# LMP88959/Digital-Subband-Video-1

Measured on AMD Instinct MI355X. Metric: encoded Mpixels/sec, 1080p 4:2:0 GOP=12, bit-exact .dsv, higher is better.
Workload: dtype u8/int16+int32 (bit-exact; packed int16 inside a proven range, int32 escape)

## Files before the change

### digital-subband-video-1_amd/csrc/dsvg_dev.hpp

```cpp
#pragma once
#include <hip/hip_runtime.h>
#include <stdint.h>
#include <stddef.h>

#define DSVG_RSU(x, s) (((x) + (1 << (s)) - 1) >> (s))

#define DSVG_GLOBAL __attribute__((address_space(1)))
template <typename T> static __device__ __forceinline__ DSVG_GLOBAL T *dsvg_global(T *p) { return (DSVG_GLOBAL T *)p; }
template <typename T> static __device__ __forceinline__ T dsvg_at(const DSVG_GLOBAL T *base, unsigned idx)
{
    return *reinterpret_cast<const DSVG_GLOBAL T *>(reinterpret_cast<const DSVG_GLOBAL char *>(base) + idx * (unsigned)sizeof(T));
}
typedef unsigned dsvg_u32x2 __attribute__((ext_vector_type(2)));
typedef unsigned dsvg_u32x4 __attribute__((ext_vector_type(4)));
template <typename P> static __device__ __forceinline__ uint2 dsvg_ld2(P p) { const dsvg_u32x2 v = *reinterpret_cast<const DSVG_GLOBAL dsvg_u32x2 *>(p); return make_uint2(v.x, v.y); }
template <typename P> static __device__ __forceinline__ void dsvg_st2(P p, uint2 v) { *reinterpret_cast<DSVG_GLOBAL dsvg_u32x2 *>(p) = dsvg_u32x2{v.x, v.y}; }
typedef unsigned dsvg_u32x4a4 __attribute__((ext_vector_type(4), aligned(4)));
typedef unsigned dsvg_u32x3a4 __attribute__((ext_vector_type(3), aligned(4)));
template <typename P> static __device__ __forceinline__ uint4 dsvg_ld4(P p) { const dsvg_u32x4 v = *reinterpret_cast<const DSVG_GLOBAL dsvg_u32x4 *>(p); return make_uint4(v.x, v.y, v.z, v.w); }
template <typename P> static __device__ __forceinline__ void dsvg_st4(P p, uint4 v) { *reinterpret_cast<DSVG_GLOBAL dsvg_u32x4 *>(p) = dsvg_u32x4{v.x, v.y, v.z, v.w}; }

struct DMV {
    int16_t x, y;
    uint8_t mode, submask, lo_var, lo_tex, high_detail, pad[3];
// ... 53 lines not shown
    unsigned long long total_bits;
    unsigned nruns;
    int dc;
    int overflow;
    int last_chunk;
    int rc;
};
static_assert(sizeof(HzPlaneSum) == 32, "HzPlaneSum travels to the host as 32-byte records");

struct HzParseChunk {
    unsigned long long m0, m1;
    int cbase;
    int prev_end;
};

struct JobDev {
    const uint8_t *src;
    const uint8_t *srcp[3];
    int srcs[3];
    const uint8_t *ref;
    uint8_t *recon;
    uint8_t *xf;
    uint8_t *pred;
    int32_t *coef;
    int32_t *s3, *s1, *s5;
    const DMV *mvs;
    const uint8_t *stable;
    int32_t *nzpos, *nzval;
    HzChunkSum *chunks;
    HzPlaneSum *psum;
    uint8_t *bits;
    size_t bits_off[3], bits_cap[3];
    size_t nz_off[3];
    size_t hz_coef_off[3];
    int chunk_off[3];
    int dec_cnt[3];
    int dec_runs[3], dec_len[3], dec_dc[3];
    long long dec_bitpos[3];
    uint8_t *nzf;
    HzParseChunk *dec_meta[3];
    long long dec_s0[3];
    int dec_npass[3], dec_ncode[3], dec_first_bad[3];
    int16_t *sym;
    uint8_t *pflag;
    uint8_t *cflag;
    unsigned *stat;
    int dec_sym[3];
    int *dec_flag;
    int dec_lim[16];
    int pf_off[3];
    int fused;
    int32_t *llsym;
    int ll_off[3];
    int llq;
    short ext[8];
    HzPlane hz[3];
    int hqp[16];
    int isP;
    int quant;
// ... 186 lines not shown
```

### digital-subband-video-1_amd/csrc/dsvg_pipe.hip

```cpp
#include <stdlib.h>
#include <algorithm>
#include <cstddef>
#include "dsvg_host.hpp"
#include "dsvg_batch_plan.h"
#include <ctime>
extern "C" void dsv1_par_for(int S, void (*fn)(void *ctx, int s, int tid), void *ctx);
extern "C" void dsv1_par_for_long(int S, void (*fn)(void *ctx, int s, int tid), void *ctx);

#define OPCHK(x) do { int rc_ = (x); if (rc_) return rc_; } while (0)

__global__ void k_spin(long long ticks)
{
    const long long t0 = wall_clock64();
    while (wall_clock64() - t0 < ticks) __builtin_amdgcn_s_sleep(16);
}
static bool streams_concurrent(hipStream_t a, hipStream_t b, hipEvent_t e0, hipEvent_t ea, hipEvent_t eb)
{
    const long long T = 10000;
    if (hipEventRecord(e0, a) != hipSuccess || hipStreamWaitEvent(b, e0, 0) != hipSuccess) return true;
    hipLaunchKernelGGL(k_spin, dim3(1), dim3(64), 0, a, T);
    hipLaunchKernelGGL(k_spin, dim3(1), dim3(64), 0, b, T);
    (void)hipEventRecord(ea, a); (void)hipEventRecord(eb, b);
    (void)hipEventSynchronize(ea); (void)hipEventSynchronize(eb);
    float ta = 0, tb = 0;
// ... 96 lines not shown
    Slab src[6], recon, xf, pred;
    int32_t *coef = nullptr, *s3 = nullptr, *s1 = nullptr, *s5 = nullptr, *nzpos = nullptr, *nzval = nullptr;
    HzChunkSum *chunks = nullptr;
    uint8_t *nzf = nullptr;
    int16_t *sym = nullptr;
    std::vector<hipEvent_t> ev_fetch;
    std::vector<short> slot_ext;
    bool no_lazy_border = false;
    bool no_list_pack = false;
    int32_t *llsym = nullptr;
    int ll_off[3] = {0, 0, 0};
    size_t ll_total = 0;
    bool llq = true;
    int16_t *symP = nullptr;
    uint8_t *pflag = nullptr;
    uint8_t *cflag = nullptr;
    unsigned *stat = nullptr;
    bool stats_on = false;
    bool no_patch_kernel = false;
    bool no_dec_sym_I = false;
    bool no_dec_sym = false;
    bool dec_sym_ok[2] = {false, false};
    HzPlaneSum *psum = nullptr;
    uint8_t *bits = nullptr;
    DMV *mvs = nullptr;
    uint8_t *stable = nullptr;
    JobDev *jobs_d = nullptr, *jobs_h = nullptr;
    std::vector<char> slot_isP;
    struct Quality {
        bool on = false;
// ... 203 lines not shown
    if (c->slot_y_d) (void)hipFree(c->slot_y_d);
    if (c->slot_y_h) (void)hipHostFree(c->slot_y_h);
    if (c->slot_cu_d) (void)hipFree(c->slot_cu_d);
    if (c->slot_cv_d) (void)hipFree(c->slot_cv_d);
    if (c->slot_cs_d) (void)hipFree(c->slot_cs_d);
    if (c->slot_cu_h) (void)hipHostFree(c->slot_cu_h);
    if (c->slot_cv_h) (void)hipHostFree(c->slot_cv_h);
    if (c->slot_cs_h) (void)hipHostFree(c->slot_cs_h);
    if (c->dec_flag_d) (void)hipFree(c->dec_flag_d);
    if (c->dec_flag_h) (void)hipHostFree(c->dec_flag_h);
    for (int i = 0; i < 6; i++) c->src[i].release();
    c->recon.release(); c->xf.release(); c->pred.release();
    xres_geo_free(c->xg);
    scale_geo_free(c->osc);
    void *d[] = {c->coef, c->s3, c->s1, c->s5, c->sym, c->nzpos, c->nzval, c->chunks, c->psum, c->bits, c->mvs, c->stable,
                 c->jobs_d, c->mvf, c->aux_tex, c->aux_var, c->csum, c->slots_d, c->luma_sums, c->yuv_stage, c->gtab_d, c->gath_d, c->ltab_d, c->otab_d, c->ingest[0], c->ingest[1], c->dec_d[0], c->dec_d[1], c->dec_meta, c->ilist_d, c->draw_scratch, c->osc_scratch, c->osc_tab_d, c->nzf, c->symP, c->pflag, c->cflag, c->stat, c->llsym, c->rc_state_d, c->rcj_d, (void *)c->xref_d};
    for (void *p : d) if (p) (void)hipFree(p);
    void *hh[] = {c->jobs_h, c->bits_h, c->psum_h, c->mv_h, c->stable_h, c->slots_h, c->luma_h, c->dec_h[0], c->dec_h[1], c->ilist_h, c->gtab_h, c->gath_h, c->aslots_h, c->amv_h, c->rcj_h, (void *)c->xref_h};
    for (void *p : hh) if (p) (void)hipHostFree(p);
    for (auto &q : c->q) { if (q.dev) (void)hipFree(q.dev); if (q.host) (void)hipHostFree(q.host); }
    if (c->st) (void)hipStreamDestroy(c->st);
    for (int i = 0; i < 2; i++) if (c->ev_mark[i]) (void)hipEventDestroy(c->ev_mark[i]);
    if (c->st_l && c->st_l != c->st_a) (void)hipStreamDestroy(c->st_l);
    if (c->ev_l) (void)hipEventDestroy(c->ev_l);
    if (c->st_a) (void)hipStreamDestroy(c->st_a);
    for (int g = 0; g < DSVG_MAX_CODE_STREAMS; g++) {
        if (c->stx[g]) (void)hipStreamDestroy(c->stx[g]);
        if (c->ev_join[g]) (void)hipEventDestroy(c->ev_join[g]);
    }
    if (c->ev_fork) (void)hipEventDestroy(c->ev_fork);
    for (hipEvent_t e : c->ev_fetch) (void)hipEventDestroy(e);
// ... 244 lines not shown
    if ((rc = c->xf.alloc(c->L[0].pitch * (size_t)max_jobs + 4096))) return fail(rc);
    if ((rc = c->pred.alloc(c->L[0].pitch * (size_t)max_jobs + 4096))) return fail(rc);
    const size_t J = (size_t)max_jobs, O = (size_t)out_slots, S = J * (size_t)c->nwin;
    if ((rc = dmalloc(&c->coef, CL.total * J, true))) return fail(rc);
    if ((rc = dmalloc(&c->s3, CL.s3total * J, true))) return fail(rc);
    if ((rc = dmalloc(&c->s1, CL.s1total * J, true))) return fail(rc);
    if ((rc = dmalloc(&c->s5, CL.s5total * J, true))) return fail(rc);
    if ((rc = dmalloc(&c->nzpos, c->nz_total * J, false))) return fail(rc);
    if ((rc = dmalloc(&c->nzval, c->nz_total * J, false))) return fail(rc);
    if ((rc = dmalloc(&c->chunks, (size_t)c->chunks_per_job * J, true))) return fail(rc);
    if ((rc = dmalloc(&c->sym, c->nz_total * J, true))) return fail(rc);
    const size_t DT = 1;
    if ((rc = dmalloc(&c->nzf, (c->nz_total >> 2) * J * DT, true))) return fail(rc);
    if ((rc = dmalloc(&c->symP, c->nz_total * J * DT, true))) return fail(rc);
    if ((rc = dmalloc(&c->pflag, CL.s3total * J, true))) return fail(rc);
    if ((rc = dmalloc(&c->cflag, (size_t)c->chunks_per_job * J * DT, true))) return fail(rc);
    {
        size_t o = 0;
        for (int p = 0; p < 3; p++) { c->ll_off[p] = (int)o; o += ((size_t)CL.w3[p] * CL.h3[p] + 7) & ~(size_t)7; }
        c->ll_total = o;
        if ((rc = dmalloc(&c->llsym, c->ll_total * J * DT, true))) return fail(rc);
    }
    c->llq = !getenv("DSV1_NO_LLQ");
    if ((rc = dmalloc(&c->stat, 8 * 64, true))) return fail(rc);
    if ((rc = dmalloc(&c->psum, 3 * O, true))) return fail(rc);
    if ((rc = dmalloc(&c->bits, c->bits_per_job * O, true))) return fail(rc);
    if ((rc = dmalloc(&c->mvs, (size_t)c->nblk * O, true))) return fail(rc);
    if ((rc = dmalloc(&c->stable, (size_t)c->nblk * O, true))) return fail(rc);
    if ((rc = dmalloc(&c->jobs_d, O, true))) return fail(rc);
    c->rc_slots = c->bgeo.rc_slots;
// ... 661 lines not shown
            dsvg_ctx *c = B.c;
            const BatchPlan &P = *B.P;
            const int k = idx % P.njobs, d = P.base + idx;
            const dsvg_pic_job &j = B.jobs[idx - k + P.order[(size_t)idx]];
            const int isP = j.ref_recon_slot >= 0;
            JobDev &jb = c->jobs_h[d];
            fill_job(c, jb, k, isP, j.quant, d);
            jb.fused = 1;
            jb.llq = c->llq ? 1 : 0;
            const size_t kk = (size_t)k;
            jb.llsym = c->llsym + kk * c->ll_total;
            for (int p = 0; p < 3; p++) jb.ll_off[p] = c->ll_off[p];
            jb.cflag = c->cflag + kk * c->chunks_per_job;
            jb.nzf = isP ? c->nzf + kk * (c->nz_total >> 2) : nullptr;
            if (isP) jb.sym = c->symP + kk * c->nz_total;
            jb.psum = c->psum + (size_t)j.out_slot * 3;
            jb.bits = c->bits + (size_t)j.out_slot * c->bits_per_job;
            jb.src = c->src[0].p + (size_t)j.src_slot * c->L[0].pitch;
            jb.srcp[0] = jb.src + c->L[0].off[0]; jb.srcs[0] = c->L[0].stride[0];
            if (c->slot_y[(size_t)j.src_slot]) { jb.srcp[0] = c->slot_y[(size_t)j.src_slot]; jb.srcs[0] = c->L[0].w[0]; }
            jb.srcp[1] = c->slot_cu[(size_t)j.src_slot]; jb.srcp[2] = c->slot_cv[(size_t)j.src_slot]; jb.srcs[1] = jb.srcs[2] = c->slot_cs[(size_t)j.src_slot];
            jb.ref = isP ? c->recon.p + (size_t)j.ref_recon_slot * c->L[0].pitch : nullptr;
            jb.recon = j.recon_slot >= 0 ? c->recon.p + (size_t)j.recon_slot * c->L[0].pitch : nullptr;
            if (isP && jb.recon && j.recon_slot != j.ref_recon_slot && !c->no_inplace_pred) jb.pred = jb.recon;
            const size_t um = (size_t)P.base + (size_t)P.mvu[(size_t)idx], us = (size_t)P.base + (size_t)P.stu[(size_t)idx];
            jb.mvs = c->mvs + um * c->nblk;
            jb.stable = c->stable + us * c->nblk;
            if (P.stcp[(size_t)idx]) memcpy(c->stable_h + us * c->nblk, j.stable_blocks, (size_t)c->nblk);
            if (P.mvcp[(size_t)idx]) memcpy(c->mv_h + um * c->nblk, j.mvs, (size_t)c->nblk * sizeof(DMV));
            memcpy(jb.ext, &P.ext[(size_t)idx * 8], sizeof(short) * 8);
// ... 881 lines not shown
```

### digital-subband-video-1_amd/csrc/k_sbt.hip

```cpp
#include <type_traits>
#include "dsvg_dev.hpp"
#include <algorithm>
#include "dsvg_kernels.hpp"
#include "dsvg_host.hpp"

template <int M>
static __device__ __forceinline__ void store_row(int32_t *p, const int (&v)[M], int n)
{
    if (n >= M) {
        if (M == 4 && (((uintptr_t)p) & 15) == 0) {
            *reinterpret_cast<int4 *>(p) = make_int4(v[0], v[1 % M], v[2 % M], v[3 % M]);
            return;
        }
        if (M == 2 && (((uintptr_t)p) & 7) == 0) {
            *reinterpret_cast<int2 *>(p) = make_int2(v[0], v[1 % M]);
            return;
        }
#pragma unroll
        for (int i = 0; i < M; i++) p[i] = v[i];
    } else {
#pragma unroll
        for (int i = 0; i < M; i++)
            if (i < n) p[i] = v[i];
    }
}

struct QCtx {
    const HzPlane *hp;
    const DSVG_GLOBAL uint8_t *stable;
    DSVG_GLOBAL int16_t *sym;
    bool any_ov;
    DSVG_GLOBAL uint8_t *nzf = nullptr, *cfl = nullptr;
    mutable int nz_any = 0;
    __device__ __forceinline__ void put_sparse(int pos, int v) const
    {
        sym[pos] = (int16_t)v;
        nzf[pos >> 2] = 1;
        cfl[pos >> 11] = 1;
    }
};
static_assert(HZ_CHUNK == 2048, "cfl index");
struct QLevel {
    int qp;
    int sh0, sh1;
    int dbx, dby, sw, base0, base1, base2;
};
template <int HZL>
static __device__ __forceinline__ QLevel q_level(const HzPlane &hp)
{
    const HzRegion &r = hp.r[1 + 3 * HZL];
    QLevel L;
    L.qp = r.qp; L.sh0 = r.qp; L.sh1 = r.qp_h;
    L.dbx = r.dbx; L.dby = r.dby; L.sw = r.sw;
    L.base0 = r.base; L.base1 = hp.r[2 + 3 * HZL].base; L.base2 = hp.r[3 + 3 * HZL].base;
    return L;
// ... 230 lines not shown
        }
        if (rowok) {
            const int pr = cy * L.sw + cx0;
            if (q.nzf) {
                int any = 0;
#pragma unroll
                for (int i = 0; i < M; i++) any |= (i < nR ? slh[i] : 0) | ((hasB && i < nC) ? shl[i] : 0) | ((hasB && i < nR) ? shh[i] : 0);
                if (any) {
                    q.nz_any = 1;
#pragma unroll
                    for (int i = 0; i < M; i++) {
                        if (i < nR && slh[i] != 0) q.put_sparse(L.base0 + pr + i, slh[i]);
                        if (hasB && i < nC && shl[i] != 0) q.put_sparse(L.base1 + pr + i, shl[i]);
                        if (hasB && i < nR && shh[i] != 0) q.put_sparse(L.base2 + pr + i, shh[i]);
                    }
                }
            } else {
                store_sym_row<M>(q.sym + L.base0 + pr, slh, nR);
                if (hasB) {
                    store_sym_row<M>(q.sym + L.base1 + pr, shl, nC);
                    store_sym_row<M>(q.sym + L.base2 + pr, shh, nR);
                }
            }
        }
    }
};
template <int N, int HZL>
static __device__ __forceinline__ void haar_fwd_patch_q(const int (&in)[N][N], int (&out)[N / 2][N / 2],
                                                        int cx0, int cy0, int ws, int hs, int W,
                                                        int wo, int ho, int32_t *__restrict__ coef, bool scaled,
// ... 32 lines not shown
            a[r][i + 4] = (int)((v.y >> (8 * i)) & 0xff) - 128;
        }
    }
    const int W = g.W, H = g.H;
    const int wo1 = DSVG_RSU(W, 1), ho1 = DSVG_RSU(H, 1), wo2 = DSVG_RSU(W, 2), ho2 = DSVG_RSU(H, 2);
    int l1[4][4], l2[2][2], l3[1][1];
    QCtx q;
    if (Q) {
        const HzPlane &hp = jb.hz[c];
        q.hp = &hp; q.stable = dsvg_global(jb.stable);
        q.sym = dsvg_global(jb.sym + jb.nz_off[c]);
        q.any_ov = (2 * hp.s_w[0] > hp.s_w[1]) || (2 * hp.s_h[0] > hp.s_h[1]) ||
                   (2 * hp.s_w[1] > hp.s_w[2]) || (2 * hp.s_h[1] > hp.s_h[2]);
        q.nzf = jb.nzf ? dsvg_global(jb.nzf + (jb.nz_off[c] >> 2)) : nullptr;
        q.cfl = jb.nzf ? dsvg_global(jb.cflag + jb.chunk_off[c]) : nullptr;
    }
    if (Q) {
        haar_fwd_patch_q<8, 2>(a, l1, 4 * I, 4 * J, W, H, W, wo1, ho1, coef, false, q);
        haar_fwd_patch_q<4, 1>(l1, l2, 2 * I, 2 * J, wo1, ho1, W, wo2, ho2, coef, true, q);
        haar_fwd_patch_q<2, 0>(l2, l3, I, J, wo2, ho2, W, g.w3, g.h3, coef, true, q);
    } else {
        haar_fwd_patch<8>(a, l1, 4 * I, 4 * J, W, H, W, wo1, ho1, coef, false);
        haar_fwd_patch<4>(l1, l2, 2 * I, 2 * J, wo1, ho1, W, wo2, ho2, coef, true);
        haar_fwd_patch<2>(l2, l3, I, J, wo2, ho2, W, g.w3, g.h3, coef, true);
    }
    jb.s3[g.s3off + (size_t)J * g.w3 + I] = l3[0][0];
    if (Q && jb.nzf) jb.pflag[g.s3off + (size_t)J * g.w3 + I] = (uint8_t)q.nz_any;
}

struct __attribute__((aligned(4))) U4A4 { unsigned x, y, z, w; };

typedef short s16x2 __attribute__((ext_vector_type(2)));
static __device__ __forceinline__ s16x2 pk2(int a, int b) { return s16x2{(short)a, (short)b}; }
static __device__ __forceinline__ s16x2 pk_min(s16x2 a, s16x2 b) { return __builtin_elementwise_min(a, b); }
static __device__ __forceinline__ s16x2 pk_max(s16x2 a, s16x2 b) { return __builtin_elementwise_max(a, b); }
static __device__ __forceinline__ s16x2 pk_rdiv2(s16x2 v) { return (v + (short)1 + (v >> 15)) >> 1; }
static __device__ __forceinline__ s16x2 pk_rdiv4(s16x2 v) { return (v + (short)2 + (v >> 15)) >> 2; }
static __device__ __forceinline__ s16x2 pk_div4(s16x2 v) { return (v + ((v >> 15) & (short)3)) >> 2; }
struct PkRow { s16x2 e0, e1, o0, o1; };
static __device__ __forceinline__ s16x2 pk_u(unsigned v) { return __builtin_bit_cast(s16x2, v); }
static __device__ __forceinline__ unsigned pk_b(s16x2 v) { return __builtin_bit_cast(unsigned, v); }
#define PK_EVEN(hi_, lo_) pk_u((lo_) & 0x00ff00ffu)
// ... 265 lines not shown
    int slh[4], shl[4], shh[4], any = 0;
#pragma unroll
    for (int i = 0; i < 4; i++) {
        const int s0 = r0[2 * i] + r0[2 * i + 1], s1 = r1[2 * i] + r1[2 * i + 1];
        const int d0 = r0[2 * i] - r0[2 * i + 1], d1 = r1[2 * i] - r1[2 * i + 1];
        out[i] = s0 + s1;
        slh[i] = sym_shift(d0 + d1, sh1); shl[i] = sym_shift(s0 - s1, sh1); shh[i] = sym_shift(d0 - d1, sh1);
        any |= slh[i] | shl[i] | shh[i];
    }
    if (any) {
        q.nz_any = 1;
        const int pr = cy1 * L1.sw + cx1;
        put_row4(q, L1.base0 + pr, slh[0], slh[1], slh[2], slh[3]);
        put_row4(q, L1.base1 + pr, shl[0], shl[1], shl[2], shl[3]);
        put_row4(q, L1.base2 + pr, shh[0], shh[1], shh[2], shh[3]);
    }
}
static __device__ __forceinline__ void fwd_fast_rows1_pk(const QCtx &q, const QLevel &L1, int sh1, int cx1, int cy1,
                                                         const PkRow &r0, const PkRow &r1, int (&out)[4])
{
    const s16x2 s0a = r0.e0 + r0.o0, s0b = r0.e1 + r0.o1, d0a = r0.e0 - r0.o0, d0b = r0.e1 - r0.o1;
    const s16x2 s1a = r1.e0 + r1.o0, s1b = r1.e1 + r1.o1, d1a = r1.e0 - r1.o0, d1b = r1.e1 - r1.o1;
    const s16x2 lla = s0a + s1a, llb = s0b + s1b;
    const s16x2 lha = d0a + d1a, lhb = d0b + d1b, hla = s0a - s1a, hlb = s0b - s1b, hha = d0a - d1a, hhb = d0b - d1b;
    out[0] = lla.x; out[1] = lla.y; out[2] = llb.x; out[3] = llb.y;
    const s16x2 mx = pk_max(pk_max(pk_max(lha, lhb), pk_max(hla, hlb)), pk_max(hha, hhb));
    const s16x2 mn = pk_min(pk_min(pk_min(lha, lhb), pk_min(hla, hlb)), pk_min(hha, hhb));
    const s16x2 am = pk_max(mx, s16x2{0, 0} - mn);
    if ((pk_b(am) & ~(((1u << min(sh1, 15)) - 1u) * 0x00010001u)) == 0) return;
    q.nz_any = 1;
    const int pr = cy1 * L1.sw + cx1;
    const short ms = (short)((1 << sh1) - 1), ss = (short)sh1;
    const s16x2 mm = {ms, ms}, sv = {ss, ss}, s15 = {15, 15};
    auto pks = [&](s16x2 v) { return (v + ((v >> s15) & mm)) >> sv; };
    put_row4(q, L1.base0 + pr, pks(lha), pks(lhb));
    put_row4(q, L1.base1 + pr, pks(hla), pks(hlb));
    put_row4(q, L1.base2 + pr, pks(hha), pks(hhb));
}
template <int N, int HZL>
static __device__ __forceinline__ void fwd_fast_level(const QCtx &q, const QLevel &L, const int (&qqv)[N / 2], const float (&rcv)[N / 2], int cx0, int cy0,
                                                      const int (&in)[N][N], int (&out)[N / 2][N / 2])
{
#pragma unroll
    for (int j = 0; j < N / 2; j++)
#pragma unroll
        for (int i = 0; i < N / 2; i++) {
            const int qq = qqv[j];
            const float rc = rcv[j];
            const int a = in[2 * j][2 * i], b = in[2 * j][2 * i + 1], c = in[2 * j + 1][2 * i], d = in[2 * j + 1][2 * i + 1];
            const int s0 = a + b, s1 = c + d, d0 = a - b, d1 = c - d;
            out[j][i] = d_ll_down(s0 + s1);
            const int vlh = d0 + d1, vhl = s0 - s1, vhh = d0 - d1;
#ifndef FWD_FAST_NO_QTEST
            if (max(max(max(vlh, vhl), vhh), -min(min(vlh, vhl), vhh)) < qq) continue;
#endif
            int slh, shl, shh;
            (void)q_coef<HZL>(qq, rc, vlh, slh);
            (void)q_coef<HZL>(qq, rc, vhl, shl);
            (void)q_coef<HZL>(qq, rc, vhh, shh);
            if (slh | shl | shh) {
                q.nz_any = 1;
                const int pr = (cy0 + j) * L.sw + cx0 + i;
                if (slh) q.put_sparse(L.base0 + pr, slh);
                if (shl) q.put_sparse(L.base1 + pr, shl);
                if (shh) q.put_sparse(L.base2 + pr, shh);
            }
        }
}

#ifndef FWD_FAST_INTRA
#define FWD_FAST_INTRA 1
#endif
struct FwdFastSel { bool ok, intra; QLevel L1, L2, L3; int i1[4], i2[2], i3; };
struct FwdFastHp { QLevel L1, L2, L3; int nbh; bool ovx, ovy, sparse; };
static __device__ __forceinline__ FwdFastHp fwd_fast_hp(const JobDev &jb, const HzPlane &hp)
{
    FwdFastHp H;
    const int sw0 = hp.s_w[0], sw1 = hp.s_w[1], sw2 = hp.s_w[2], sh0 = hp.s_h[0], sh1 = hp.s_h[1], sh2 = hp.s_h[2];
    H.L1 = q_level<2>(hp); H.L2 = q_level<1>(hp); H.L3 = q_level<0>(hp);
    H.nbh = hp.nbh;
// ... 55 lines not shown
    FWD_PIN(H.L1.sh0); FWD_PIN(H.L1.sh1); FWD_PIN(H.L1.dbx); FWD_PIN(H.L1.dby); FWD_PIN(H.L2.qp); FWD_PIN(H.L2.dbx); FWD_PIN(H.L2.dby);
    FWD_PIN(H.L3.qp); FWD_PIN(H.L3.dbx); FWD_PIN(H.L3.dby); FWD_PIN(H.nbh); FWD_PIN(mvtab); FWD_PIN(stable_p); FWD_PIN(srcp_p); FWD_PIN(sstride);
#endif
    DMV mv;
    {
        const auto mq = reinterpret_cast<const DSVG_GLOBAL char *>(dsvg_global(mvs0 ? mvs0 + (size_t)job * nblk : mvtab)) + (unsigned)blk * (unsigned)sizeof(DMV);
        const unsigned xy = *reinterpret_cast<const DSVG_GLOBAL unsigned *>(mq);
        mv.x = (int16_t)(xy & 0xffffu); mv.y = (int16_t)(xy >> 16); mv.mode = *reinterpret_cast<const DSVG_GLOBAL uint8_t *>(mq + 4);
    }
    QCtx q;
    q.hp = &hp; q.stable = dsvg_global(stable_p);
    q.sym = dsvg_global(jb.sym + jb.nz_off[c]);
    q.any_ov = H.ovx | H.ovy;
    q.nzf = H.sparse ? dsvg_global(jb.nzf + (jb.nz_off[c] >> 2)) : nullptr;
    q.cfl = H.sparse ? dsvg_global(jb.cflag + jb.chunk_off[c]) : nullptr;
    const FwdFastSel S = fwd_fast_sel(H, mv.mode, I, J, x0, y0, pw, ph);
    if (!S.ok) return;
    const QLevel &L1 = S.L1, &L2 = S.L2, &L3 = S.L3;
    const auto sp = dsvg_global(srcp_p);
    uint2 sw[8];
    if (S.intra) {
        const auto px = dsvg_global(static_cast<const uint8_t *>(jb.xf + g.poff));
#pragma unroll
        for (int r = 0; r < 8; r++) sw[r] = dsvg_ld2(px + (unsigned)((y0 + r) * stride + x0));
    } else {
#pragma unroll
        for (int r = 0; r < 8; r++) sw[r] = dsvg_ld2(sp + (unsigned)((y0 + r) * sstride + x0));
    }
    int f1[4], f2[2];
#pragma unroll
// ... 78 lines not shown
#endif
#pragma unroll
    for (int j = 0; j < 2; j++) {
        fq.q2[j] = max(L2.qp >> ((f2[j] & 2) ? 2 : (f2[j] != 0)), HZ_MINQ);
        fq.rc2[j] = __builtin_amdgcn_rcpf((float)(fq.q2[j] << 1));
    }
    fq.q3 = max(L3.qp >> ((f3 & 2) ? 2 : (f3 != 0)), HZ_MINQ);
    fq.rc3 = __builtin_amdgcn_rcpf((float)(fq.q3 << 1));
    int l2[2][2], l3[1][1];
    fwd_fast_level<4, 1>(q, L2, fq.q2, fq.rc2, 2 * I, 2 * J, l1, l2);
    const int q3v[1] = {fq.q3};
    const float rc3v[1] = {fq.rc3};
    fwd_fast_level<2, 0>(q, L3, q3v, rc3v, I, J, l2, l3);
    dsvg_global(jb.s3 + g.s3off)[(unsigned)(J * g.w3 + I)] = l3[0][0];
    dsvg_global(jb.pflag + g.s3off)[(unsigned)(J * g.w3 + I)] = (uint8_t)q.nz_any;
}
#ifndef FAST_WPE_L
#define FAST_WPE_L 4
#endif
#ifndef FAST_WPE_C
#define FAST_WPE_C 0
#endif
#if FAST_WPE_L > 0
#define FAST_WPE_L_ATTR __attribute__((amdgpu_waves_per_eu(FAST_WPE_L, FAST_WPE_L)))
#else
#define FAST_WPE_L_ATTR
#endif
#if FAST_WPE_C > 0
#define FAST_WPE_C_ATTR __attribute__((amdgpu_waves_per_eu(FAST_WPE_C, FAST_WPE_C)))
#else
// ... 91 lines not shown
    const int bi = (int)(((float)I + 0.5f) * __builtin_amdgcn_rcpf((float)(bw >> 3)));
    const int bj = (int)(((float)J + 0.5f) * __builtin_amdgcn_rcpf((float)(bh >> 3)));
    const int nblk = MG.nbh * MG.nbv, blk = bj * MG.nbh + bi;
    const DMV mv = mvs0 ? mvs0[(size_t)job * nblk + blk] : jb.mvs[blk];
    int32_t *coef = jb.coef + g.coff;
    const int W = g.W, H = g.H;
    const int wo1 = DSVG_RSU(W, 1), ho1 = DSVG_RSU(H, 1), wo2 = DSVG_RSU(W, 2), ho2 = DSVG_RSU(H, 2);
    QCtx q;
    const HzPlane &hp = jb.hz[c];
    q.hp = &hp; q.stable = dsvg_global(jb.stable);
    q.sym = dsvg_global(jb.sym + jb.nz_off[c]);
    q.any_ov = (2 * hp.s_w[0] > hp.s_w[1]) || (2 * hp.s_h[0] > hp.s_h[1]) ||
               (2 * hp.s_w[1] > hp.s_w[2]) || (2 * hp.s_h[1] > hp.s_h[2]);
    q.nzf = jb.nzf ? dsvg_global(jb.nzf + (jb.nz_off[c] >> 2)) : nullptr;
    q.cfl = jb.nzf ? dsvg_global(jb.cflag + jb.chunk_off[c]) : nullptr;
    if (skip_fast && fwd_fast_sel(jb, hp, q.any_ov, mv.mode, I, J, x0, y0, pw, ph).ok) return;
#ifdef AB_COUNT_GENERAL
    if (jb.stat) atomicAdd(jb.stat + 64 * (2 + (c != 0)) + (threadIdx.x & 63), 1u);
#endif
    HaarQ<8, 2> hq1;
    hq1.init(q, 4 * I, 4 * J, W, H, wo1, ho1);
    int l1[4][4], ra[2][8];

    if (mv.mode != 0) {
        const auto px = dsvg_global(static_cast<const uint8_t *>(jb.xf + g.poff));
#pragma unroll
        for (int r = 0; r < 8; r++) {
            const int y = y0 + r;
            uint2 v = make_uint2(0x80808080u, 0x80808080u);
            if (y < ph) v = dsvg_ld2(px + (unsigned)(y * stride + x0));
// ... 45 lines not shown
        };
        if (CH == 0) {
            if (any_y) mc_luma_patch<true, true>(gr, stride, xh, yh, emit);
            else if (any_x) mc_luma_patch<true, false>(gr, stride, xh, yh, emit);
            else mc_luma_patch<false, false>(gr, stride, xh, yh, emit);
        } else {
            if (any_x || any_y) mc_chroma_patch<true>(gr, stride, xh, yh, emit);
            else mc_chroma_patch<false>(gr, stride, xh, yh, emit);
        }
    }
    int l2[2][2], l3[1][1];
    haar_fwd_patch_q<4, 1>(l1, l2, 2 * I, 2 * J, wo1, ho1, W, wo2, ho2, coef, true, q);
    haar_fwd_patch_q<2, 0>(l2, l3, I, J, wo2, ho2, W, g.w3, g.h3, coef, true, q);
    dsvg_global(jb.s3 + g.s3off)[(unsigned)(J * g.w3 + I)] = l3[0][0];
    if (jb.nzf) dsvg_global(jb.pflag + g.s3off)[(unsigned)(J * g.w3 + I)] = (uint8_t)q.nz_any;
}

#ifndef FWD_B4T_WPE
#define FWD_B4T_WPE 6
#endif
#if FWD_B4T_WPE
#define FWD_B4T_ATTR __attribute__((amdgpu_waves_per_eu(FWD_B4T_WPE, FWD_B4T_WPE)))
#else
#define FWD_B4T_ATTR
#endif
template <bool Q>
__global__ __launch_bounds__(256) FWD_B4T_ATTR void k_fwd_b4t(const JobDev *__restrict__ jobs, SbtGeo3 G, int c0, int npl,
                                                 int from_src)
{
    int job, c;
// ... 1555 lines not shown
            if (r >= nrow) break;
            unsigned o[2];
#pragma unroll
            for (int h = 0; h < 2; h++) {
                const unsigned pw_ = h ? pv[r].y : pv[r].x;
                const s16x2 e = cc + __builtin_bit_cast(s16x2, pw_ & 0x00ff00ffu), od = cc + __builtin_bit_cast(s16x2, __builtin_amdgcn_perm(0u, pw_, 0x0c030c01u));
                unsigned eb, ob;
                asm("v_sat_pk_u8_i16 %0, %1" : "=v"(eb) : "v"(__builtin_bit_cast(unsigned, e)));
                asm("v_sat_pk_u8_i16 %0, %1" : "=v"(ob) : "v"(__builtin_bit_cast(unsigned, od)));
                o[h] = __builtin_amdgcn_perm(ob, eb, 0x05010400u);
            }
            dsvg_st2(outp + (p0 + r * stride), make_uint2(o[0], o[1]));
        }
        return;
    }
    const HzPlane &hp = jb.hz[c];
    const auto sym = dsvg_global(static_cast<const int16_t *>(jb.sym + jb.nz_off[c]));
    const auto stb = dsvg_global(jb.stable);
    const QLevel Q3 = q_level<0>(hp), Q2 = q_level<1>(hp), Q1 = q_level<2>(hp);
    const unsigned nbh = (unsigned)hp.nbh;
    auto flag = [&](const QLevel &Q, int cx, int cy) { return (int)stb[__umul24(__umul24((unsigned)cy, (unsigned)Q.dby) >> 14, nbh) + (__umul24((unsigned)cx, (unsigned)Q.dbx) >> 14)]; };
    int l2[2][2], l1[4][4];
    {
        const int f = flag(Q3, I, J), q = max(Q3.qp >> ((f & 2) ? 2 : (f != 0)), HZ_MINQ);
        const unsigned o = (unsigned)(J * Q3.sw + I);
        const int LL = d_ll_up_t<true>(ll3), LH = dq_lo24(dsvg_at(sym, (unsigned)Q3.base0 + o), q),
                  HL = part ? 0 : dq_lo24(dsvg_at(sym, (unsigned)Q3.base1 + o), q), HH = part ? 0 : dq_lo24(dsvg_at(sym, (unsigned)Q3.base2 + o), q);
        l2[0][0] = d_div4<true>(LL + LH + HL + HH); l2[0][1] = d_div4<true>(LL - LH + HL - HH);
        l2[1][0] = d_div4<true>(LL + LH - HL - HH); l2[1][1] = d_div4<true>(LL - LH - HL + HH);
    }
#pragma unroll
    for (int j = 0; j < 2; j++)
#pragma unroll
        for (int i = 0; i < 2; i++) {
            if (part && j == 1) { l1[2][2 * i] = l1[2][2 * i + 1] = l1[3][2 * i] = l1[3][2 * i + 1] = 0; continue; }
            const int cx = 2 * I + i, cy = 2 * J + j;
            const int f = flag(Q2, cx, cy), q = max(Q2.qp >> ((f & 2) ? 2 : (f != 0)), HZ_MINQ);
            const unsigned o = (unsigned)(cy * Q2.sw + cx);
            const int LL = d_ll_up_t<true>(l2[j][i]), LH = dq_lo24(dsvg_at(sym, (unsigned)Q2.base0 + o), q), HL = dq_lo24(dsvg_at(sym, (unsigned)Q2.base1 + o), q),
                      HH = dq_lo24(dsvg_at(sym, (unsigned)Q2.base2 + o), q);
            l1[2 * j][2 * i] = d_div4<true>(LL + LH + HL + HH); l1[2 * j][2 * i + 1] = d_div4<true>(LL - LH + HL - HH);
            l1[2 * j + 1][2 * i] = d_div4<true>(LL + LH - HL - HH); l1[2 * j + 1][2 * i + 1] = d_div4<true>(LL - LH - HL + HH);
        }
#pragma unroll
    for (int j = 0; j < 4; j++) {
        if (part && j >= 2) break;
        int r0[8], r1[8];
#pragma unroll
        for (int i = 0; i < 4; i++) {
            const int cx = 4 * I + i, cy = 4 * J + j;
            const int sh = flag(Q1, cx, cy) ? Q1.sh1 : Q1.sh0;
            const unsigned o = (unsigned)(cy * Q1.sw + cx);
            const int LL = l1[j][i], LH = (int)((unsigned)(int)dsvg_at(sym, (unsigned)Q1.base0 + o) << sh), HL = (int)((unsigned)(int)dsvg_at(sym, (unsigned)Q1.base1 + o) << sh),
                      HH = (int)((unsigned)(int)dsvg_at(sym, (unsigned)Q1.base2 + o) << sh);
            r0[2 * i] = d_div4<true>(LL + LH + HL + HH); r0[2 * i + 1] = d_div4<true>(LL - LH + HL - HH);
            r1[2 * i] = d_div4<true>(LL + LH - HL - HH); r1[2 * i + 1] = d_div4<true>(LL - LH - HL + HH);
        }
#pragma unroll
        for (int rr = 0; rr < 2; rr++) {
            const int r = 2 * j + rr;
            const uint2 pw2 = dsvg_ld2(pred + (p0 + r * stride));
            unsigned lo = 0, hi = 0;
#pragma unroll
            for (int i = 0; i < 8; i++) {
                const int p = (int)(((i < 4 ? pw2.x : pw2.y) >> (8 * (i & 3))) & 0xff);
                const int sv = d_sat8(d_sat8((rr ? r1[i] : r0[i]) + 128) + p - 128);
                if (i < 4) lo |= (unsigned)sv << (8 * i); else hi |= (unsigned)sv << (8 * (i - 4));
            }
            dsvg_st2(outp + (p0 + r * stride), make_uint2(lo, hi));
        }
    }
    };
    if (I < imax && J < jmax) { if (J == jpart) run(std::true_type{}); else run(std::false_type{}); }
    if (!fb || J >= jmax) return;
    if (!(bwl || bwr || btop || bbot)) return;
    __threadfence_block();
    if (bwl || bwr) plane_sides(g, jobs[job].ext + 4, 8 * J, bnrow, 8 * imax);
    if ((btop || bbot) && I < imax) plane_tb(g, jobs[job].ext + 4, 8 * I, 1, 8 * J, bnrow);
}

#ifndef BT_CX
#define BT_CX 60
#endif
#ifndef BT_CY
#define BT_CY 32
#endif
// ... 436 lines not shown
```

Before: 238,400.

## Stash per-patch chroma symbols in contiguous record for inverse reconstruction

The forward quantize kernels now write each chroma patch's quantized subband symbols into a contiguous 128-byte per-patch record with a validity mask. The inverse/reconstruct kernel reads these records with a few vector loads instead of scattered per-coefficient gathers from the sparse symbol planes. This replaces strided gathers across three levels and three bands with coalesced reads. In exchange it adds extra stores in the forward pass and a new P-frame device buffer.

```diff
diff --git a/digital-subband-video-1_amd/csrc/dsvg_dev.hpp b/digital-subband-video-1_amd/csrc/dsvg_dev.hpp
--- a/digital-subband-video-1_amd/csrc/dsvg_dev.hpp
+++ b/digital-subband-video-1_amd/csrc/dsvg_dev.hpp
@@ -91,6 +91,7 @@
     int prev_end;
 };
 
+#define DSVG_PREC_BYTES 128
 struct JobDev {
     const uint8_t *src;
     const uint8_t *srcp[3];
@@ -120,6 +121,7 @@
     int dec_npass[3], dec_ncode[3], dec_first_bad[3];
     int16_t *sym;
     uint8_t *pflag;
+    uint8_t *prec;
     uint8_t *cflag;
     unsigned *stat;
     int dec_sym[3];
diff --git a/digital-subband-video-1_amd/csrc/dsvg_pipe.hip b/digital-subband-video-1_amd/csrc/dsvg_pipe.hip
--- a/digital-subband-video-1_amd/csrc/dsvg_pipe.hip
+++ b/digital-subband-video-1_amd/csrc/dsvg_pipe.hip
@@ -134,6 +134,8 @@
     bool llq = true;
     int16_t *symP = nullptr;
     uint8_t *pflag = nullptr;
+    uint8_t *prec = nullptr;
+    size_t prec_per_job = 0;
     uint8_t *cflag = nullptr;
     unsigned *stat = nullptr;
     bool stats_on = false;
@@ -367,7 +369,7 @@
     xres_geo_free(c->xg);
     scale_geo_free(c->osc);
     void *d[] = {c->coef, c->s3, c->s1, c->s5, c->sym, c->nzpos, c->nzval, c->chunks, c->psum, c->bits, c->mvs, c->stable,
-                 c->jobs_d, c->mvf, c->aux_tex, c->aux_var, c->csum, c->slots_d, c->luma_sums, c->yuv_stage, c->gtab_d, c->gath_d, c->ltab_d, c->otab_d, c->ingest[0], c->ingest[1], c->dec_d[0], c->dec_d[1], c->dec_meta, c->ilist_d, c->draw_scratch, c->osc_scratch, c->osc_tab_d, c->nzf, c->symP, c->pflag, c->cflag, c->stat, c->llsym, c->rc_state_d, c->rcj_d, (void *)c->xref_d};
+                 c->jobs_d, c->mvf, c->aux_tex, c->aux_var, c->csum, c->slots_d, c->luma_sums, c->yuv_stage, c->gtab_d, c->gath_d, c->ltab_d, c->otab_d, c->ingest[0], c->ingest[1], c->dec_d[0], c->dec_d[1], c->dec_meta, c->ilist_d, c->draw_scratch, c->osc_scratch, c->osc_tab_d, c->nzf, c->symP, c->pflag, c->prec, c->cflag, c->stat, c->llsym, c->rc_state_d, c->rcj_d, (void *)c->xref_d};
     for (void *p : d) if (p) (void)hipFree(p);
     void *hh[] = {c->jobs_h, c->bits_h, c->psum_h, c->mv_h, c->stable_h, c->slots_h, c->luma_h, c->dec_h[0], c->dec_h[1], c->ilist_h, c->gtab_h, c->gath_h, c->aslots_h, c->amv_h, c->rcj_h, (void *)c->xref_h};
     for (void *p : hh) if (p) (void)hipHostFree(p);
@@ -642,6 +644,8 @@
     if ((rc = dmalloc(&c->nzf, (c->nz_total >> 2) * J * DT, true))) return fail(rc);
     if ((rc = dmalloc(&c->symP, c->nz_total * J * DT, true))) return fail(rc);
     if ((rc = dmalloc(&c->pflag, CL.s3total * J, true))) return fail(rc);
+    c->prec_per_job = (CL.s3total - CL.s3off[1]) * (size_t)DSVG_PREC_BYTES;
+    if ((rc = dmalloc(&c->prec, c->prec_per_job * J, false))) return fail(rc);
     if ((rc = dmalloc(&c->cflag, (size_t)c->chunks_per_job * J * DT, true))) return fail(rc);
     {
         size_t o = 0;
@@ -1333,6 +1337,7 @@
             jb.cflag = c->cflag + kk * c->chunks_per_job;
             jb.nzf = isP ? c->nzf + kk * (c->nz_total >> 2) : nullptr;
             if (isP) jb.sym = c->symP + kk * c->nz_total;
+            if (isP) jb.prec = c->prec + kk * c->prec_per_job;
             jb.psum = c->psum + (size_t)j.out_slot * 3;
             jb.bits = c->bits + (size_t)j.out_slot * c->bits_per_job;
             jb.src = c->src[0].p + (size_t)j.src_slot * c->L[0].pitch;
diff --git a/digital-subband-video-1_amd/csrc/k_sbt.hip b/digital-subband-video-1_amd/csrc/k_sbt.hip
--- a/digital-subband-video-1_amd/csrc/k_sbt.hip
+++ b/digital-subband-video-1_amd/csrc/k_sbt.hip
@@ -38,7 +38,29 @@
         nzf[pos >> 2] = 1;
         cfl[pos >> 11] = 1;
     }
+    DSVG_GLOBAL int16_t *rec = nullptr;
+    mutable int rmask = 0;
+    __device__ __forceinline__ void rec_row1(int j, unsigned lh01, unsigned lh23, unsigned hl01, unsigned hl23, unsigned hh01, unsigned hh23) const
+    {
+        DSVG_GLOBAL int16_t *p = rec + 12 * j;
+        dsvg_st2(p, make_uint2(lh01, lh23)); dsvg_st2(p + 4, make_uint2(hl01, hl23)); dsvg_st2(p + 8, make_uint2(hh01, hh23));
+        rmask |= 1 << j;
+    }
+    template <int HZL>
+    __device__ __forceinline__ void rec_cell(int k, int slh, int shl, int shh) const
+    {
+        DSVG_GLOBAL int16_t *p = rec + (HZL == 1 ? 48 + 3 * k : 60);
+        p[0] = (int16_t)slh; p[1] = (int16_t)shl; p[2] = (int16_t)shh;
+        rmask |= HZL == 1 ? 16 << k : 256;
+    }
+    __device__ __forceinline__ void rec_close() const { if (rec && nz_any) rec[63] = (int16_t)rmask; }
 };
+static __device__ __forceinline__ unsigned rec_pk(int a, int b) { return ((unsigned)a & 0xffffu) | ((unsigned)b << 16); }
+static __device__ __forceinline__ DSVG_GLOBAL int16_t *rec_of(const JobDev &jb, const SbtGeo3 &G, int c, unsigned pidx)
+{
+    if (c == 0 || !jb.prec) return nullptr;
+    return dsvg_global(reinterpret_cast<int16_t *>(jb.prec)) + (G.g[c].s3off - G.g[1].s3off) * (DSVG_PREC_BYTES / 2) + pidx * (unsigned)(DSVG_PREC_BYTES / 2);
+}
 static_assert(HZ_CHUNK == 2048, "cfl index");
 struct QLevel {
     int qp;
@@ -299,6 +321,17 @@
                         if (hasB && i < nC && shl[i] != 0) q.put_sparse(L.base1 + pr + i, shl[i]);
                         if (hasB && i < nR && shh[i] != 0) q.put_sparse(L.base2 + pr + i, shh[i]);
                     }
+                    if (q.rec) {
+                        int a[M], b[M], c[M];
+#pragma unroll
+                        for (int i = 0; i < M; i++) { a[i] = i < nR ? slh[i] : 0; b[i] = (hasB && i < nC) ? shl[i] : 0; c[i] = (hasB && i < nR) ? shh[i] : 0; }
+                        if constexpr (HZL == 2) q.rec_row1(j, rec_pk(a[0], a[1 % M]), rec_pk(a[2 % M], a[3 % M]), rec_pk(b[0], b[1 % M]), rec_pk(b[2 % M], b[3 % M]),
+                                                           rec_pk(c[0], c[1 % M]), rec_pk(c[2 % M], c[3 % M]));
+                        else {
+#pragma unroll
+                            for (int i = 0; i < M; i++) q.template rec_cell<HZL>(2 * j + i, a[i], b[i], c[i]);
+                        }
+                    }
                 }
             } else {
                 store_sym_row<M>(q.sym + L.base0 + pr, slh, nR);
@@ -361,6 +394,7 @@
                    (2 * hp.s_w[1] > hp.s_w[2]) || (2 * hp.s_h[1] > hp.s_h[2]);
         q.nzf = jb.nzf ? dsvg_global(jb.nzf + (jb.nz_off[c] >> 2)) : nullptr;
         q.cfl = jb.nzf ? dsvg_global(jb.cflag + jb.chunk_off[c]) : nullptr;
+        q.rec = jb.nzf ? rec_of(jb, G, c, (unsigned)(J * g.w3 + I)) : nullptr;
     }
     if (Q) {
         haar_fwd_patch_q<8, 2>(a, l1, 4 * I, 4 * J, W, H, W, wo1, ho1, coef, false, q);
@@ -373,6 +407,7 @@
     }
     jb.s3[g.s3off + (size_t)J * g.w3 + I] = l3[0][0];
     if (Q && jb.nzf) jb.pflag[g.s3off + (size_t)J * g.w3 + I] = (uint8_t)q.nz_any;
+    if (Q) q.rec_close();
 }
 
 struct __attribute__((aligned(4))) U4A4 { unsigned x, y, z, w; };
@@ -668,6 +703,7 @@
         put_row4(q, L1.base0 + pr, slh[0], slh[1], slh[2], slh[3]);
         put_row4(q, L1.base1 + pr, shl[0], shl[1], shl[2], shl[3]);
         put_row4(q, L1.base2 + pr, shh[0], shh[1], shh[2], shh[3]);
+        if (q.rec) q.rec_row1(cy1 & 3, rec_pk(slh[0], slh[1]), rec_pk(slh[2], slh[3]), rec_pk(shl[0], shl[1]), rec_pk(shl[2], shl[3]), rec_pk(shh[0], shh[1]), rec_pk(shh[2], shh[3]));
     }
 }
 static __device__ __forceinline__ void fwd_fast_rows1_pk(const QCtx &q, const QLevel &L1, int sh1, int cx1, int cy1,
@@ -687,9 +723,11 @@
     const short ms = (short)((1 << sh1) - 1), ss = (short)sh1;
     const s16x2 mm = {ms, ms}, sv = {ss, ss}, s15 = {15, 15};
     auto pks = [&](s16x2 v) { return (v + ((v >> s15) & mm)) >> sv; };
-    put_row4(q, L1.base0 + pr, pks(lha), pks(lhb));
-    put_row4(q, L1.base1 + pr, pks(hla), pks(hlb));
-    put_row4(q, L1.base2 + pr, pks(hha), pks(hhb));
+    const s16x2 slha = pks(lha), slhb = pks(lhb), shla = pks(hla), shlb = pks(hlb), shha = pks(hha), shhb = pks(hhb);
+    put_row4(q, L1.base0 + pr, slha, slhb);
+    put_row4(q, L1.base1 + pr, shla, shlb);
+    put_row4(q, L1.base2 + pr, shha, shhb);
+    if (q.rec) q.rec_row1(cy1 & 3, pk_b(slha), pk_b(slhb), pk_b(shla), pk_b(shlb), pk_b(shha), pk_b(shhb));
 }
 template <int N, int HZL>
 static __device__ __forceinline__ void fwd_fast_level(const QCtx &q, const QLevel &L, const int (&qqv)[N / 2], const float (&rcv)[N / 2], int cx0, int cy0,
@@ -718,6 +756,7 @@
                 if (slh) q.put_sparse(L.base0 + pr, slh);
                 if (shl) q.put_sparse(L.base1 + pr, shl);
                 if (shh) q.put_sparse(L.base2 + pr, shh);
+                if (q.rec) q.template rec_cell<HZL>(2 * j + i, slh, shl, shh);
             }
         }
 }
@@ -803,6 +842,7 @@
     q.any_ov = H.ovx | H.ovy;
     q.nzf = H.sparse ? dsvg_global(jb.nzf + (jb.nz_off[c] >> 2)) : nullptr;
     q.cfl = H.sparse ? dsvg_global(jb.cflag + jb.chunk_off[c]) : nullptr;
+    if (CH) q.rec = H.sparse ? rec_of(jb, G, c, (unsigned)(J * g.w3 + I)) : nullptr;
     const FwdFastSel S = fwd_fast_sel(H, mv.mode, I, J, x0, y0, pw, ph);
     if (!S.ok) return;
     const QLevel &L1 = S.L1, &L2 = S.L2, &L3 = S.L3;
@@ -911,6 +951,7 @@
     fwd_fast_level<2, 0>(q, L3, q3v, rc3v, I, J, l2, l3);
     dsvg_global(jb.s3 + g.s3off)[(unsigned)(J * g.w3 + I)] = l3[0][0];
     dsvg_global(jb.pflag + g.s3off)[(unsigned)(J * g.w3 + I)] = (uint8_t)q.nz_any;
+    if (CH) q.rec_close();
 }
 #ifndef FAST_WPE_L
 #define FAST_WPE_L 4
@@ -1032,6 +1073,7 @@
                (2 * hp.s_w[1] > hp.s_w[2]) || (2 * hp.s_h[1] > hp.s_h[2]);
     q.nzf = jb.nzf ? dsvg_global(jb.nzf + (jb.nz_off[c] >> 2)) : nullptr;
     q.cfl = jb.nzf ? dsvg_global(jb.cflag + jb.chunk_off[c]) : nullptr;
+    if (CH) q.rec = jb.nzf ? rec_of(jb, G, c, (unsigned)(J * g.w3 + I)) : nullptr;
     if (skip_fast && fwd_fast_sel(jb, hp, q.any_ov, mv.mode, I, J, x0, y0, pw, ph).ok) return;
 #ifdef AB_COUNT_GENERAL
     if (jb.stat) atomicAdd(jb.stat + 64 * (2 + (c != 0)) + (threadIdx.x & 63), 1u);
@@ -1107,6 +1149,7 @@
     haar_fwd_patch_q<2, 0>(l2, l3, I, J, wo2, ho2, W, g.w3, g.h3, coef, true, q);
     dsvg_global(jb.s3 + g.s3off)[(unsigned)(J * g.w3 + I)] = l3[0][0];
     if (jb.nzf) dsvg_global(jb.pflag + g.s3off)[(unsigned)(J * g.w3 + I)] = (uint8_t)q.nz_any;
+    if (CH) q.rec_close();
 }
 
 #ifndef FWD_B4T_WPE
@@ -2692,18 +2735,35 @@
         }
         return;
     }
+    auto flagged = [&](auto REC_) {
+    constexpr bool REC = decltype(REC_)::value;
     const HzPlane &hp = jb.hz[c];
     const auto sym = dsvg_global(static_cast<const int16_t *>(jb.sym + jb.nz_off[c]));
+    const auto rec = dsvg_global(reinterpret_cast<const int16_t *>(jb.prec)) + (g.s3off - G.g[1].s3off) * (DSVG_PREC_BYTES / 2) + pidx * (unsigned)(DSVG_PREC_BYTES / 2);
     const auto stb = dsvg_global(jb.stable);
     const QLevel Q3 = q_level<0>(hp), Q2 = q_level<1>(hp), Q1 = q_level<2>(hp);
     const unsigned nbh = (unsigned)hp.nbh;
     auto flag = [&](const QLevel &Q, int cx, int cy) { return (int)stb[__umul24(__umul24((unsigned)cy, (unsigned)Q.dby) >> 14, nbh) + (__umul24((unsigned)cx, (unsigned)Q.dbx) >> 14)]; };
+    auto lo16 = [](unsigned w) { return (int)(w << 16) >> 16; };
+    auto hi16 = [](unsigned w) { return (int)w >> 16; };
     int l2[2][2], l1[4][4];
+    unsigned rm = 0, w2[6] = {0u, 0u, 0u, 0u, 0u, 0u};
     {
         const int f = flag(Q3, I, J), q = max(Q3.qp >> ((f & 2) ? 2 : (f != 0)), HZ_MINQ);
         const unsigned o = (unsigned)(J * Q3.sw + I);
-        const int LL = d_ll_up_t<true>(ll3), LH = dq_lo24(dsvg_at(sym, (unsigned)Q3.base0 + o), q),
-                  HL = part ? 0 : dq_lo24(dsvg_at(sym, (unsigned)Q3.base1 + o), q), HH = part ? 0 : dq_lo24(dsvg_at(sym, (unsigned)Q3.base2 + o), q);
+        int s0, s1, s2;
+        if constexpr (REC) {
+            const uint2 t = dsvg_ld2(rec + 60);
+            const uint4 a = dsvg_ld4(rec + 48);
+            const uint2 b = dsvg_ld2(rec + 56);
+            w2[0] = a.x; w2[1] = a.y; w2[2] = a.z; w2[3] = a.w; w2[4] = b.x; w2[5] = b.y;
+            rm = t.y >> 16;
+            const bool v = (rm & 256u) != 0;
+            s0 = v ? lo16(t.x) : 0; s1 = (v && !part) ? hi16(t.x) : 0; s2 = (v && !part) ? lo16(t.y) : 0;
+        } else {
+            s0 = dsvg_at(sym, (unsigned)Q3.base0 + o); s1 = part ? 0 : (int)dsvg_at(sym, (unsigned)Q3.base1 + o); s2 = part ? 0 : (int)dsvg_at(sym, (unsigned)Q3.base2 + o);
+        }
+        const int LL = d_ll_up_t<true>(ll3), LH = dq_lo24(s0, q), HL = part ? 0 : dq_lo24(s1, q), HH = part ? 0 : dq_lo24(s2, q);
         l2[0][0] = d_div4<true>(LL + LH + HL + HH); l2[0][1] = d_div4<true>(LL - LH + HL - HH);
         l2[1][0] = d_div4<true>(LL + LH - HL - HH); l2[1][1] = d_div4<true>(LL - LH - HL + HH);
     }
@@ -2715,8 +2775,17 @@
             const int cx = 2 * I + i, cy = 2 * J + j;
             const int f = flag(Q2, cx, cy), q = max(Q2.qp >> ((f & 2) ? 2 : (f != 0)), HZ_MINQ);
             const unsigned o = (unsigned)(cy * Q2.sw + cx);
-            const int LL = d_ll_up_t<true>(l2[j][i]), LH = dq_lo24(dsvg_at(sym, (unsigned)Q2.base0 + o), q), HL = dq_lo24(dsvg_at(sym, (unsigned)Q2.base1 + o), q),
-                      HH = dq_lo24(dsvg_at(sym, (unsigned)Q2.base2 + o), q);
+            int s0, s1, s2;
+            if constexpr (REC) {
+                const int n = 3 * (2 * j + i);
+                const bool v = (rm >> (4 + 2 * j + i)) & 1u;
+                s0 = v ? ((n & 1) ? hi16(w2[n >> 1]) : lo16(w2[n >> 1])) : 0;
+                s1 = v ? (((n + 1) & 1) ? hi16(w2[(n + 1) >> 1]) : lo16(w2[(n + 1) >> 1])) : 0;
+                s2 = v ? (((n + 2) & 1) ? hi16(w2[(n + 2) >> 1]) : lo16(w2[(n + 2) >> 1])) : 0;
+            } else {
+                s0 = dsvg_at(sym, (unsigned)Q2.base0 + o); s1 = dsvg_at(sym, (unsigned)Q2.base1 + o); s2 = dsvg_at(sym, (unsigned)Q2.base2 + o);
+            }
+            const int LL = d_ll_up_t<true>(l2[j][i]), LH = dq_lo24(s0, q), HL = dq_lo24(s1, q), HH = dq_lo24(s2, q);
             l1[2 * j][2 * i] = d_div4<true>(LL + LH + HL + HH); l1[2 * j][2 * i + 1] = d_div4<true>(LL - LH + HL - HH);
             l1[2 * j + 1][2 * i] = d_div4<true>(LL + LH - HL - HH); l1[2 * j + 1][2 * i + 1] = d_div4<true>(LL - LH - HL + HH);
         }
@@ -2724,13 +2793,23 @@
     for (int j = 0; j < 4; j++) {
         if (part && j >= 2) break;
         int r0[8], r1[8];
+        uint2 wl = make_uint2(0u, 0u), wh = wl, wd = wl;
+        if constexpr (REC) {
+            if ((rm >> j) & 1u) { wl = dsvg_ld2(rec + 12 * j); wh = dsvg_ld2(rec + 12 * j + 4); wd = dsvg_ld2(rec + 12 * j + 8); }
+        }
 #pragma unroll
         for (int i = 0; i < 4; i++) {
             const int cx = 4 * I + i, cy = 4 * J + j;
             const int sh = flag(Q1, cx, cy) ? Q1.sh1 : Q1.sh0;
             const unsigned o = (unsigned)(cy * Q1.sw + cx);
-            const int LL = l1[j][i], LH = (int)((unsigned)(int)dsvg_at(sym, (unsigned)Q1.base0 + o) << sh), HL = (int)((unsigned)(int)dsvg_at(sym, (unsigned)Q1.base1 + o) << sh),
-                      HH = (int)((unsigned)(int)dsvg_at(sym, (unsigned)Q1.base2 + o) << sh);
+            int s0, s1, s2;
+            if constexpr (REC) {
+                const unsigned a = i < 2 ? wl.x : wl.y, b = i < 2 ? wh.x : wh.y, d = i < 2 ? wd.x : wd.y;
+                s0 = (i & 1) ? hi16(a) : lo16(a); s1 = (i & 1) ? hi16(b) : lo16(b); s2 = (i & 1) ? hi16(d) : lo16(d);
+            } else {
+                s0 = dsvg_at(sym, (unsigned)Q1.base0 + o); s1 = dsvg_at(sym, (unsigned)Q1.base1 + o); s2 = dsvg_at(sym, (unsigned)Q1.base2 + o);
+            }
+            const int LL = l1[j][i], LH = (int)((unsigned)s0 << sh), HL = (int)((unsigned)s1 << sh), HH = (int)((unsigned)s2 << sh);
             r0[2 * i] = d_div4<true>(LL + LH + HL + HH); r0[2 * i + 1] = d_div4<true>(LL - LH + HL - HH);
             r1[2 * i] = d_div4<true>(LL + LH - HL - HH); r1[2 * i + 1] = d_div4<true>(LL - LH - HL + HH);
         }
@@ -2748,6 +2827,8 @@
             dsvg_st2(outp + (p0 + r * stride), make_uint2(lo, hi));
         }
     }
+    };
+    if (c != 0 && jb.prec) flagged(std::true_type{}); else flagged(std::false_type{});
     };
     if (I < imax && J < jmax) { if (J == jpart) run(std::true_type{}); else run(std::false_type{}); }
     if (!fb || J >= jmax) return;
```

New measurement: 235,500. 0.988x the previous value.
